# stelleg/caster-dta

Measured on AMD Instinct MI355X. Metric: graph-pairs/sec (Davis-shaped protein+drug), encoders fwd+bwd, higher is better.
Workload: dtype f32; 1 GPU; davis_b64; pairs_per_gpu=64, residues_per_gpu=19200, protein_edges_per_gpu=57484, atoms_per_gpu=2560, drug_edges_per_gpu=7986, encoder=CASTER-DTA(2,2), pass=fwdbwd, activation_storage=fp32, scope=encoders, torch_compile=False, tunable_gemms=False, two_lane_head=False, train_mode=True, csr_build_in_step=True, hip_graph=True, kernels=mfma

## Files before the change

caster-dta_amd/csrc/gvp_internal.h:

```cpp
#pragma once
#include <hip/hip_runtime.h>
#include <stdint.h>

#include "../../include/caster_gvp.h"
#include "gvp_math.h"
#include "gvp_rng.h"

constexpr int POLICY_F32 = 0, POLICY_BF16 = 1, POLICY_GVPDEF = 2, POLICY_LINEAR = 3;

struct QuadOffsets {
  int emb, conv0, node0, layer_stride, head, total;
  int embT, convT0, nodeT0, layerT_stride, headT;
};

#ifndef CGVP_BWD_MAX_GRID
#define CGVP_BWD_MAX_GRID 240
#endif
constexpr int kBwdMaxGrid = CGVP_BWD_MAX_GRID;

#include <atomic>
#include <type_traits>

template <auto Kernel, class... A>
int launch_reserving(dim3 grid, dim3 block, size_t lds, size_t reserve, hipStream_t st, const A&... args) {
// ... 14 lines not shown
  return 0;
}
template <auto Kernel, class... A>
int launch(dim3 grid, dim3 block, size_t lds, hipStream_t st, const A&... args) {
  return launch_reserving<Kernel>(grid, block, lds, lds, st, args...);
}

namespace gq { struct bf16s; struct f32_gvpdef; struct f32_linear; }
template <class T> struct Tag { using type = T; };
template <class ST> constexpr bool is_layer_kind = std::is_same_v<ST, gq::f32_gvpdef> || std::is_same_v<ST, gq::f32_linear>;
template <bool KINDS, class F>
int with_policy(int policy, F&& f) {
  if (policy == POLICY_F32) return f(Tag<float>{});
  if (policy == POLICY_BF16) return f(Tag<gq::bf16s>{});
  if constexpr (KINDS) {
    if (policy == POLICY_GVPDEF) return f(Tag<gq::f32_gvpdef>{});
    if (policy == POLICY_LINEAR) return f(Tag<gq::f32_linear>{});
  }
  return CGVP_ERR_UNSUPPORTED_DIMS;
}
template <class F>
int with_flag(bool b, F&& f) { return b ? f(std::true_type{}) : f(std::false_type{}); }

namespace quad {
int offsets(int nt_node, int nt_edge, int num_convs, QuadOffsets* o);
int prepare(const gvp::EncLayout& L, int num_convs, int packed_bf16, const float* params, float* image, hipStream_t st);
int node_embed(int nt_node, const float* img, const float* x_s, const float* x_v, const int64_t* ntypes,
               int64_t N, float* h, unsigned long long* rng_state, unsigned long long* rng_out, int policy, hipStream_t st);
int pass_begin(const gvp::EncLayout& L, int num_convs, int policy, const float* params, float* image, const float* x_s,
               const float* x_v, const int64_t* ntypes, int64_t N, float* h, unsigned long long* rng_state,
               unsigned long long* rng_out, const int64_t* edge_index, int64_t E, int32_t* counters, hipStream_t st);
int conv(int nt_edge, const float* img, const float* h, const float* e_s, const float* e_v,
         const int64_t* etypes, const int32_t* rowptr, const int32_t* eperm, const int32_t* esrc,
         const int32_t* edst, int64_t N, int64_t E, int mean, float* dh, int fuse, const float* img_node,
         const float* img_head, float* h_out, float* out, const float* mask0, const float* mask1, gvp::RngArgs rng,
         const float* e_in, float* e_out, int policy, hipStream_t st);
int node_update(const float* img_node, const float* img_head, const float* h, const float* dh, int64_t N,
                int with_head, float* h_out, float* out, const float* mask0, const float* mask1, gvp::RngArgs rng,
                int policy, hipStream_t st);

int node_update_bwd(const float* img_node, const float* imgT_node, const float* h, const float* dh,
                    const float* mask0, const float* mask1, gvp::RngArgs rng, const float* g_up0, const float* g_up1,
                    const float* g_up2, int64_t N, float* g_dh, float* g_h, float* zero_rows, float* slab, int* grid,
                    int policy, hipStream_t st);
int head_bwd(const float* img_head, const float* imgT_head, const float* h_out, const float* g_out, int64_t N,
             float* g_h_out, float* slab, int* grid, int policy, hipStream_t st);
int node_head_bwd(const float* img_head, const float* imgT_head, const float* h_out, const float* g_out, float* g_h_out,
                  float* head_slab, const float* img_node, const float* imgT_node, const float* h, const float* dh,
                  const float* mask0, const float* mask1, gvp::RngArgs rng, int64_t N, float* g_dh, float* g_h,
                  float* zero_rows, float* slab, int* grid, int policy, hipStream_t st);
int conv_bwd(int nt_edge, const float* img, const float* imgT, const float* h, const float* e_emb,
             const int32_t* rowptr, const int32_t* esrc, const int32_t* edst, int64_t N, int64_t E, int mean,
             const float* g_dh, float* g_src, float* g_dst, float* g_e, float* slab, int* grid, int policy, hipStream_t st,
             float* g_edge = nullptr, float* slot = nullptr);
// ... 44 lines not shown
```

caster-dta_amd/csrc/gvp_kernels.hip:

```cpp
#include <hip/hip_runtime.h>
#include <stdlib.h>
#include <stdint.h>

#include "gvp_internal.h"

using namespace gvp;

namespace {

constexpr int WAVE = 64;

inline int check_dims(const cgvp_dims* d) {
  if (!d) return CGVP_ERR_BAD_ARG;
  if (d->node_in_s != NODE_IN_S || d->node_in_v != NODE_IN_V || d->edge_in_s != EDGE_IN_S ||
      d->edge_in_v != EDGE_IN_V || d->hidden_s != NS || d->hidden_v != NV ||
      d->edge_hidden_s != ES || d->edge_hidden_v != EV || d->out_s != OUT)
    return CGVP_ERR_UNSUPPORTED_DIMS;
  if (d->storage != CGVP_F32 && d->storage != CGVP_BF16) return CGVP_ERR_UNSUPPORTED_DIMS;
  if (d->layer_kind < CGVP_LAYER_GATED || d->layer_kind > CGVP_LAYER_LINEAR) return CGVP_ERR_UNSUPPORTED_DIMS;
  if (d->layer_kind != CGVP_LAYER_GATED && d->storage != CGVP_F32) return CGVP_ERR_UNSUPPORTED_DIMS;
  return 0;
}
inline int check_dims_gated(const cgvp_dims* d) {
  if (int rc = check_dims(d)) return rc;
// ... 21 lines not shown

struct BwdLookup : QuadOffsets { quad::BwdBlocks blk; };
inline int bwd_lookup(const cgvp_layout& l, BwdLookup* o) {
  if (int rc = quad::offsets(l.nt_node, l.nt_edge, num_convs_of(l), o)) return rc;
  return quad::bwd_block_sizes(l.nt_node, l.nt_edge, &o->blk);
}
inline int emit_segments(const cgvp_segment* sg, int n, cgvp_segment* segs, int32_t* nsegs, float* grad_params,
                         hipStream_t st, int overwrite = 0, bool store_only = false) {
  if (segs && nsegs) { for (int k = 0; k < n; ++k) segs[k] = sg[k]; *nsegs = n; }
  else quad::reduce_segments(sg, n, grad_params, st, overwrite, store_only);
  return launch_status();
}

__global__ void zero_words_kernel(uint32_t* __restrict__ p, size_t n) {
  for (size_t i = (size_t)blockIdx.x * blockDim.x + threadIdx.x; i < n; i += (size_t)gridDim.x * blockDim.x) p[i] = 0u;
}
inline void zero_words(void* p, size_t words, hipStream_t s) {
  if (words == 0 || !p) return;
  size_t blocks = (words + 1023) / 1024;
  if (blocks > 2048) blocks = 2048;
  hipLaunchKernelGGL(zero_words_kernel, dim3((unsigned)blocks), dim3(256), 0, s, reinterpret_cast<uint32_t*>(p), words);
}

__global__ void csr_count_kernel(const int64_t* __restrict__ ei, int64_t N, int64_t E,
                                 int32_t* __restrict__ cnt, unsigned long long* rng_state, unsigned long long* rng_out) {
  int64_t e = (int64_t)blockIdx.x * blockDim.x + threadIdx.x;
  if (rng_state && e == 0) {
    const unsigned long long off = rng_state[1] + 1;
    rng_state[1] = off;
    rng_out[0] = rng_state[0];
    rng_out[1] = off;
  }
  if (e >= E) return;
  int64_t s = ei[e], d = ei[E + e];
  if (s < 0 || s >= N || d < 0 || d >= N) return;
  atomicAdd(&cnt[d], 1);
}

constexpr int SCAN_LDS = 36 * 1024;
__global__ __launch_bounds__(1024) void csr_scan_kernel(const int32_t* __restrict__ cnt, int64_t N,
                                                        int32_t* __restrict__ rowptr) {
  extern __shared__ int32_t sbuf[];
  const int t = threadIdx.x;
  const int tile_cap = (int)(N < SCAN_LDS ? (N + 3) / 4 * 4 : SCAN_LDS);
  int32_t* part = sbuf + tile_cap;
  int32_t carry = 0;
  for (int64_t base = 0; base < N || base == 0; base += SCAN_LDS) {
    const int64_t rem = N - base;
    const int n = (int)(rem < SCAN_LDS ? (rem > 0 ? rem : 0) : SCAN_LDS);
    constexpr int VPT = SCAN_LDS / 4096;
    int4 v[VPT];
    const int n4 = n >> 2;
    const int4* src4 = reinterpret_cast<const int4*>(cnt + base);
#pragma unroll
    for (int k = 0; k < VPT; ++k) {
      const int q = t + 1024 * k;
      v[k] = q < n4 ? src4[q] : make_int4(0, 0, 0, 0);
    }
#pragma unroll
// ... 26 lines not shown
    }
    __syncthreads();
    const int32_t wave_base = (t >> 6) > 0 ? part[16 + (t >> 6) - 1] : 0;
    const int32_t total = part[31];
    int32_t run = carry + wave_base + inc - sum;
    for (int i = lo; i < hi; ++i) { const int32_t c = sbuf[i]; sbuf[i] = run; run += c; }
    __syncthreads();
    if ((((uintptr_t)(rowptr + base)) & 15) == 0) {
      for (int q = t; q < n4; q += 1024) {
        const int4 x = reinterpret_cast<const int4*>(sbuf)[q];
        reinterpret_cast<int4*>(rowptr + base)[q] = x;
      }
      if (t < (n & 3)) rowptr[base + (n4 << 2) + t] = sbuf[(n4 << 2) + t];
    } else {
      for (int i = t; i < n; i += 1024) rowptr[base + i] = sbuf[i];
    }
    carry += total;
    __syncthreads();
    if (N == 0) break;
  }
  if (t == 0) rowptr[N] = carry;
}

constexpr int SCAN_MULTI_MAX = 65536, SCAN_MULTI_T = 256, SCAN_MULTI_CHUNK = 4 * SCAN_MULTI_T;
__global__ __launch_bounds__(SCAN_MULTI_T) void csr_scan_multi_kernel(const int32_t* __restrict__ cnt, int32_t N,
                                                                      int32_t counters, int32_t* __restrict__ rowptr) {
  __shared__ int32_t part[2 * (SCAN_MULTI_T / WAVE)];
  const int t = threadIdx.x, wv = t >> 6;
  const int4* c4 = reinterpret_cast<const int4*>(cnt);
  int32_t pre = 0;
  for (int q = t; q < (int)blockIdx.x * SCAN_MULTI_T; q += SCAN_MULTI_T) {
    const int4 v = c4[q];
    pre += (v.x + v.y) + (v.z + v.w);
  }
  const int i0 = (int)blockIdx.x * SCAN_MULTI_CHUNK + 4 * t;
  const int4 v = i0 < counters ? c4[i0 >> 2] : make_int4(0, 0, 0, 0);
  const int32_t sum = (v.x + v.y) + (v.z + v.w);
  int32_t inc = sum;
#pragma unroll
  for (int off = 1; off < WAVE; off <<= 1) {
    const int32_t u = __shfl_up(inc, off);
    if ((t & (WAVE - 1)) >= off) inc += u;
    pre += __shfl_xor(pre, off);
  }
  if ((t & (WAVE - 1)) == WAVE - 1) { part[wv] = inc; part[SCAN_MULTI_T / WAVE + wv] = pre; }
  __syncthreads();
  int32_t run = inc - sum;
// ... 21 lines not shown
  tmp[pos] = (int32_t)e;
  edst[pos] = (int32_t)d;
}

__global__ void csr_rank_kernel(const int64_t* __restrict__ ei, int64_t N, int64_t E, int64_t counters,
                                const int32_t* __restrict__ rowptr, const int32_t* __restrict__ tmp,
                                int32_t* __restrict__ edst, int32_t* __restrict__ eperm,
                                int32_t* __restrict__ esrc, int32_t* __restrict__ cnt) {
  const int64_t t = (int64_t)blockIdx.x * blockDim.x + threadIdx.x;
  if (t < counters) cnt[t] = 0;
  if (t >= rowptr[N] || t >= E) {
    if (t < E) { eperm[t] = -1; esrc[t] = 0; edst[t] = 0; }
    return;
  }
  const int32_t n = edst[t];
  if (n < 0 || n >= N) return;
  int32_t lo = rowptr[n], hi = rowptr[n + 1];
  const int32_t key = tmp[t];
  if (lo < 0 || hi > E || lo > hi || key < 0 || key >= E) return;
  int32_t rank = 0;
  for (int32_t j = lo; j < hi; ++j) rank += tmp[j] < key ? 1 : 0;
  eperm[lo + rank] = key;
  esrc[lo + rank] = (int32_t)ei[key];
}

__global__ void src_count_kernel(const int32_t* __restrict__ esrc, const int32_t* __restrict__ rowptr, int64_t N,
                                 int32_t* __restrict__ cnt) {
  const int64_t p = (int64_t)blockIdx.x * blockDim.x + threadIdx.x;
  if (p >= rowptr[N]) return;
  const int32_t s = esrc[p];
  if (s >= 0 && s < N) atomicAdd(&cnt[s], 1);
}
__global__ void src_fill_kernel(const int32_t* __restrict__ esrc, const int32_t* __restrict__ rowptr, int64_t N,
                                const int32_t* __restrict__ sptr, int32_t* __restrict__ cnt, int32_t* __restrict__ tmp) {
  const int64_t p = (int64_t)blockIdx.x * blockDim.x + threadIdx.x;
  const int32_t ev = rowptr[N];
  if (p >= ev) return;
  const int32_t s = esrc[p];
  if (s < 0 || s >= N) return;
  const int32_t pos = sptr[s] + atomicSub(&cnt[s], 1) - 1;
  if (pos >= 0 && pos < ev) tmp[pos] = (int32_t)p;
}
__global__ void src_rank_kernel(const int32_t* __restrict__ esrc, const int32_t* __restrict__ rowptr, int64_t N,
                                const int32_t* __restrict__ sptr, const int32_t* __restrict__ tmp, int32_t* __restrict__ spos) {
  const int64_t k = (int64_t)blockIdx.x * blockDim.x + threadIdx.x;
  const int32_t ev = rowptr[N];
// ... 370 lines not shown
    if (a.width == 20) {
      if (blk < 4) {
        float fs[4], fv;
        gvp::dropout_row20(a.rng.seed[0], a.rng.seed[1], a.rng.stream + m, n, blk, a.rng.p, fs, fv);
        row[4 * blk] = fs[0]; row[4 * blk + 1] = fs[1]; row[4 * blk + 2] = fs[2]; row[4 * blk + 3] = fs[3];
        row[16 + blk] = fv;
      }
    } else {
      float f[4];
      gvp::dropout4(a.rng.seed[0], a.rng.seed[1], a.rng.stream + m, n, blk, a.rng.p, f);
      row[4 * blk] = f[0]; row[4 * blk + 1] = f[1]; row[4 * blk + 2] = f[2]; row[4 * blk + 3] = f[3];
    }
  }
}

extern "C" {

int cgvp_abi_version(void) { return CGVP_ABI_VERSION; }
const char* cgvp_build_info(void) { return "libcaster_gvp gfx950 (HIP, wave64), built " __DATE__ " " __TIME__; }

int cgvp_csr_from_coo(const int64_t* edge_index, int64_t N, int64_t E, int32_t* rowptr,
                      int32_t* eperm, int32_t* esrc, int32_t* edst, int32_t* work, int32_t work_is_zero,
                      int32_t* ids_scratch, void* stream) {
  return quad::csr_build(edge_index, N, E, rowptr, eperm, esrc, edst, work, work_is_zero, ids_scratch, nullptr, nullptr,
                         (hipStream_t)stream);
}
}

namespace quad {
void zero_words(void* p, size_t words, hipStream_t s) { ::zero_words(p, words, s); }

int csr_build(const int64_t* edge_index, int64_t N, int64_t E, int32_t* rowptr, int32_t* eperm, int32_t* esrc,
              int32_t* edst, int32_t* work, int work_is_zero, int32_t* ids_scratch, unsigned long long* rng_state,
              unsigned long long* rng_out, hipStream_t stream) {
  if (N < 0 || E < 0 || !rowptr || !work || (E > 0 && (!edge_index || !eperm || !esrc || !edst || !ids_scratch)))
    return CGVP_ERR_BAD_ARG;
  if (N >= (int64_t)1 << 31 || E >= (int64_t)1 << 31) return CGVP_ERR_BAD_ARG;
  if ((uintptr_t)work & 15) return CGVP_ERR_BAD_ARG;
  hipStream_t s = stream;
  const int64_t counters = (N + 1 + 63) / 64 * 64;
  if (work_is_zero == 0) {
    zero_words(work, (size_t)counters, s);
  }
  int32_t* tmp = ids_scratch;
  const int B = 256;
  if (E > 0 && work_is_zero != 2)
    hipLaunchKernelGGL(csr_count_kernel, dim3((unsigned)((E + B - 1) / B)), dim3(B), 0, s, edge_index, N, E, work, rng_state, rng_out);
  else if (rng_state)
    hipLaunchKernelGGL(rng_next_kernel, dim3(1), dim3(1), 0, s, rng_state, rng_out);
  if (N < SCAN_MULTI_MAX) {
    hipLaunchKernelGGL(csr_scan_multi_kernel, dim3((unsigned)((N + 1 + SCAN_MULTI_CHUNK - 1) / SCAN_MULTI_CHUNK)),
                       dim3(SCAN_MULTI_T), 0, s, work, (int32_t)N, (int32_t)counters, rowptr);
  } else {
    const int64_t tile = N < SCAN_LDS ? (N + 3) / 4 * 4 : SCAN_LDS;
    hipLaunchKernelGGL(csr_scan_kernel, dim3(1), dim3(1024), (size_t)(tile + 1024 + 32) * sizeof(int32_t), s, work, N, rowptr);
  }
  if (E > 0) hipLaunchKernelGGL(csr_fill_kernel, dim3((unsigned)((E + B - 1) / B)), dim3(B), 0, s, edge_index, N, E, rowptr, work, tmp, edst);
  const int64_t span = E > counters ? E : counters;
  hipLaunchKernelGGL(csr_rank_kernel, dim3((unsigned)((span + B - 1) / B)), dim3(B), 0, s, edge_index, N, E, counters, rowptr, tmp,
                     edst, eperm, esrc, work);
  return launch_status();
}

bool deterministic_env() {
  static const bool v = [] { const char* e = getenv("CGVP_DETERMINISTIC"); return e && e[0] == '1'; }();
  return v;
}

int64_t src_index_work_ints(int64_t N, int64_t E) { return (N + 1 + 63) / 64 * 64 + (E > 0 ? E : 1); }

int src_index(const int32_t* rowptr, const int32_t* esrc, int64_t N, int64_t E, int32_t* sptr, int32_t* spos,
              int32_t* work, hipStream_t s) {
  if (N < 0 || E < 0 || !rowptr || !sptr || !work || (E > 0 && (!esrc || !spos))) return CGVP_ERR_BAD_ARG;
  if (N >= (int64_t)1 << 31 || E >= (int64_t)1 << 31 || ((uintptr_t)work & 15)) return CGVP_ERR_BAD_ARG;
  const int64_t counters = (N + 1 + 63) / 64 * 64;
  int32_t* cnt = work;
  int32_t* tmp = work + counters;
  zero_words(cnt, (size_t)counters, s);
  const int B = 256;
  const unsigned eb = (unsigned)((E + B - 1) / B);
// ... 41 lines not shown
  return 0;
}

int64_t cgvp_lba_image_floats(const cgvp_dims* dims, const cgvp_layout* layout) {
  if (int rc = check_dims(dims)) return rc;
  if (!layout) return CGVP_ERR_BAD_ARG;
  QuadOffsets o;
  if (int rc = quad::offsets(layout->nt_node, layout->nt_edge, num_convs_of(*layout), &o)) return rc;
  return o.total;
}

int cgvp_lba_prepare(const cgvp_dims* dims, const cgvp_layout* layout, const float* params, float* image,
                     void* stream) {
  if (int rc = check_dims(dims)) return rc;
  if (!layout || !params || !image) return CGVP_ERR_BAD_ARG;
  if (int rc = quad::prepare(cvt(*layout), num_convs_of(*layout), policy_of(dims) == POLICY_BF16 ? 1 : 0, params, image, (hipStream_t)stream)) return rc;
  return launch_status();
}

int cgvp_lba_pass_begin(const cgvp_dims* dims, const cgvp_layout* layout, const float* params, float* image,
                        const float* x_s, const float* x_v, const int64_t* ntypes, int64_t N, float* h,
                        uint64_t* rng_state, uint64_t* rng_out, const int64_t* edge_index, int64_t E,
                        int32_t* csr_counters, void* stream) {
  if (int rc = check_dims_gated(dims)) return rc;
  if (N < 0 || E < 0 || !layout || !params || !image || (layout->nt_node > 0 && N > 0 && !ntypes)) return CGVP_ERR_BAD_ARG;
  if ((rng_state != nullptr) != (rng_out != nullptr)) return CGVP_ERR_BAD_ARG;
  if (((uintptr_t)rng_state & 7) || ((uintptr_t)rng_out & 7) || ((uintptr_t)h & 15) || ((uintptr_t)image & 15)) return CGVP_ERR_BAD_ARG;
  if ((edge_index != nullptr) != (csr_counters != nullptr)) return CGVP_ERR_BAD_ARG;
  if (N > 0 && (!x_s || !x_v || !h)) return CGVP_ERR_BAD_ARG;
  if (N >= (int64_t)1 << 31 || E >= (int64_t)1 << 31) return CGVP_ERR_BAD_ARG;
  if (N == 0 && rng_state)
    if (int rc = cgvp_rng_next(rng_state, rng_out, stream)) return rc;
  if (int rc = quad::pass_begin(cvt(*layout), num_convs_of(*layout), policy_of(dims), params, image, x_s, x_v, ntypes, N, h,
                                reinterpret_cast<unsigned long long*>(rng_state), reinterpret_cast<unsigned long long*>(rng_out),
                                edge_index, E, csr_counters, (hipStream_t)stream)) return rc;
  return launch_status();
}


int cgvp_node_embed_fwd(const cgvp_dims* dims, const cgvp_layout* layout, const float* params,
                        const float* image, const float* x_s, const float* x_v, const int64_t* ntypes,
                        int64_t N, float* h, uint64_t* rng_state, uint64_t* rng_out, void* stream) {
  if (int rc = check_dims_gated(dims)) return rc;
  if (N < 0 || !layout || !params || (layout->nt_node > 0 && N > 0 && !ntypes)) return CGVP_ERR_BAD_ARG;
  if ((rng_state != nullptr) != (rng_out != nullptr) || (rng_state && !image)) return CGVP_ERR_BAD_ARG;
  if (((uintptr_t)rng_state & 7) || ((uintptr_t)rng_out & 7)) return CGVP_ERR_BAD_ARG;
  if (N == 0) return rng_state ? cgvp_rng_next(rng_state, rng_out, stream) : 0;
  if (!x_s || !x_v || !h) return CGVP_ERR_BAD_ARG;
  if (image) {
    if ((uintptr_t)h & 15) return CGVP_ERR_BAD_ARG;
    QuadOffsets o;
    if (int rc = quad::offsets(layout->nt_node, layout->nt_edge, num_convs_of(*layout), &o)) return rc;
    if (int rc = quad::node_embed(layout->nt_node, image + o.emb, x_s, x_v, ntypes, N, h,
                                  reinterpret_cast<unsigned long long*>(rng_state),
                                  reinterpret_cast<unsigned long long*>(rng_out), policy_of(dims), (hipStream_t)stream)) return rc;
    return launch_status();
  }
  if (policy_of(dims)) return CGVP_ERR_UNSUPPORTED_DIMS;
  NodeEmbedArgs a{params, cvt(*layout), x_s, x_v, ntypes, N, h};
  const dim3 grid((unsigned)((N + WAVE - 1) / WAVE));
  hipStream_t st = (hipStream_t)stream;
// ... 380 lines not shown
```

caster-dta_amd/csrc/gvp_quad_kernels.hip:

```cpp
#include <hip/hip_runtime.h>
#include <stdlib.h>
#include <stdint.h>

#include "gvp_internal.h"
#include "gvp_quad.h"

using namespace gq;

namespace {

#ifdef CGVP_STAMPS
__device__ unsigned long long* g_stamp_buf = nullptr;
#define STAMP(slot)                                                                          \
  do {                                                                                       \
    __builtin_amdgcn_sched_barrier(0);                                                       \
    unsigned long long t_;                                                                   \
    asm volatile("s_waitcnt vmcnt(0) lgkmcnt(0)\n\ts_memtime %0\n\ts_waitcnt lgkmcnt(0)" : "=s"(t_)::"memory"); \
    __builtin_amdgcn_sched_barrier(0);                                                       \
    if (g_stamp_buf && (threadIdx.x & 63) == 0)                                              \
      g_stamp_buf[((size_t)blockIdx.x * WPB + (threadIdx.x >> 6)) * 16 + (slot)] = t_;        \
  } while (0)
#define STAMP_REAL(slot)                                                                     \
  do {                                                                                       \
    unsigned long long t_;                                                                   \
// ... 124 lines not shown
  int type[1] = {0};
#pragma unroll
  for (int s = 0; s < Q::SSTEPS; ++s) {
    const int c = 4 * s + g;
    bs[0][s] = (active && c < NODE_IN_S) ? Io<ST>::ld(a.x_s, n * NODE_IN_S + c) : 0.f;
  }
#pragma unroll
  for (int p = 0; p < 3; ++p) bv[0][p][0] = (active && g < NODE_IN_V) ? Io<ST>::ld(a.x_v, n * 3 * NODE_IN_V + 3 * g + p) : 0.f;
  if (NTN > 0 && active) {
    type[0] = (int)a.ntypes[n];
    type[0] = type[0] < 0 ? 0 : (type[0] >= NTN ? NTN - 1 : type[0]);
  }
  f4 s[1][1];
  float v[1][3][1];
  typename Q::Cache c[1];
  Q::template forward<1, Io<ST>::BF>(lds + IM::EMB_GVP, lane, type, bs, bv, s, v, c);
  ln_quad<NS, NV>(lds + IM::EMB_LN, lane, s[0], v[0]);
  if (active) {
    Io<ST>::st4(a.h, n * ROW + 4 * g, s[0][0]);
#pragma unroll
    for (int p = 0; p < 3; ++p) Io<ST>::st(a.h, n * ROW + NS + 3 * g + p, v[0][p][0]);
  }
}
__device__ __forceinline__ void rng_handoff(const EmbedQArgs& a) {
  if (a.rng_state && blockIdx.x == 0 && threadIdx.x == 0) {
    const unsigned long long off = a.rng_state[1] + 1;
    a.rng_state[1] = off;
    a.rng_out[0] = a.rng_state[0];
    a.rng_out[1] = off;
  }
}

template <int NTN, typename ST>
__global__ __launch_bounds__(TPB) void embed_quad_kernel(EmbedQArgs a) {
  typedef Image<NTN, 0> IM;
  __shared__ __attribute__((aligned(16))) float lds[IM::EMB_SIZE];
  stage_slice<IM::EMB_SIZE>(lds, a.img, threadIdx.x);
  rng_handoff(a);
  __syncthreads();
  embed_tile<NTN, ST>(a, lds, blockIdx.x);
}

struct PassBeginArgs {
  EmbedQArgs e;
  const float* params; EncLayout L; int num_convs; int packed; float* image;
  const int64_t* ei; int64_t E; int64_t Ncount; int32_t* counters;
  int embed_blocks, prep_blocks;
};
template <int NTN, int NTE, typename ST>
__global__ __launch_bounds__(TPB) void pass_begin_kernel(PassBeginArgs a) {
  typedef Image<NTN, NTE> IM;
  __shared__ __attribute__((aligned(16))) float lds[IM::EMB_SIZE];
  const int b = blockIdx.x;
  if (b >= a.embed_blocks + a.prep_blocks) {
    const int64_t e = (int64_t)(b - a.embed_blocks - a.prep_blocks) * TPB + threadIdx.x;
    if (e < a.E) {
      const int64_t s = a.ei[e], d = a.ei[a.E + e];
      if (s >= 0 && s < a.Ncount && d >= 0 && d < a.Ncount) atomicAdd(&a.counters[d], 1);
    }
    return;
  }
  if (b >= a.embed_blocks) {
    const int total = IM::total(a.num_convs);
    for (int idx = (b - a.embed_blocks) * TPB + threadIdx.x; idx < total; idx += a.prep_blocks * TPB)
      a.image[idx] = image_element<NTN, NTE>(a.params, a.L, a.num_convs, a.packed, idx);
    return;
  }
  for (int k = threadIdx.x; k < IM::EMB_SIZE; k += TPB) lds[k] = image_element<NTN, NTE>(a.params, a.L, a.num_convs, a.packed, k);
  rng_handoff(a.e);
  __syncthreads();
  embed_tile<NTN, ST>(a.e, lds, b);
}

struct NodeQArgs {
  const float* img_node; const float* img_head;
  const float* h; const float* dh; int64_t N; float* h_out; float* out;
  const float* mask0; const float* mask1;
  gvp::RngArgs rng;
};
constexpr int MROW = NS + NV;

__device__ __forceinline__ void node_dropout(const float* mask, const gvp::RngArgs& rng, int which, int64_t n, int g,
                                             f4& ms, float& mv) {
  if (mask) {
    ms = *reinterpret_cast<const f4*>(mask + n * MROW + 4 * g);
    mv = mask[n * MROW + NS + g];
  } else if (rng.seed) {
    const unsigned long long seed = rng.seed[0], off = rng.seed[1];
    float fs[4];
    gvp::dropout_row20(seed, off, rng.stream + which, n, g, rng.p, fs, mv);
    ms = f4{fs[0], fs[1], fs[2], fs[3]};
  }
// ... 414 lines not shown
int node_embed(int nt_node, const float* img, const float* x_s, const float* x_v, const int64_t* ntypes,
               int64_t N, float* h, unsigned long long* rng_state, unsigned long long* rng_out, int policy, hipStream_t st) {
  EmbedQArgs a{img, x_s, x_v, ntypes, N, h, rng_state, rng_out};
  const dim3 grid((unsigned)((N + WPB * TILE - 1) / (WPB * TILE)));
  return with_policy<false>(policy, [&](auto tag) {
    using ST = typename decltype(tag)::type;
    switch (nt_node) {
      case 0: return launch<embed_quad_kernel<0, ST>>(grid, dim3(TPB), 0, st, a);
      case 20: return launch<embed_quad_kernel<20, ST>>(grid, dim3(TPB), 0, st, a);
      case 21: return launch<embed_quad_kernel<21, ST>>(grid, dim3(TPB), 0, st, a);
      default: return CGVP_ERR_UNSUPPORTED_DIMS;
    }
  });
}

template <int NTN, int NTE>
int pass_begin_impl(const PassBeginArgs& a, int blocks, int policy, hipStream_t st) {
  return with_policy<false>(policy, [&](auto tag) {
    return launch<pass_begin_kernel<NTN, NTE, typename decltype(tag)::type>>(dim3(blocks), dim3(TPB), 0, st, a);
  });
}
int pass_begin(const EncLayout& L, int num_convs, int policy, const float* params, float* image, const float* x_s,
               const float* x_v, const int64_t* ntypes, int64_t N, float* h, unsigned long long* rng_state,
               unsigned long long* rng_out, const int64_t* edge_index, int64_t E, int32_t* counters, hipStream_t st) {
  QuadOffsets o;
  if (int rc = offsets(L.nt_node, L.nt_edge, num_convs, &o)) return rc;
  PassBeginArgs a{};
  a.e = EmbedQArgs{nullptr, x_s, x_v, ntypes, N, h, rng_state, rng_out};
  a.params = params; a.L = L; a.num_convs = num_convs; a.packed = policy == POLICY_BF16 ? 1 : 0; a.image = image;
  a.ei = edge_index; a.E = (edge_index && counters) ? E : 0; a.Ncount = N; a.counters = counters;
  a.embed_blocks = (int)((N + WPB * TILE - 1) / (WPB * TILE));
  a.prep_blocks = (o.total + TPB - 1) / TPB;
  const int blocks = a.embed_blocks + a.prep_blocks + (int)((a.E + TPB - 1) / TPB);
  return with_nt(L.nt_node, L.nt_edge, [&](auto ntn, auto nte) {
    return pass_begin_impl<decltype(ntn)::value, decltype(nte)::value>(a, blocks, policy, st);
  });
}

inline int conv_fwd_waves(int64_t groups) {
  static const int forced = [] { const char* e = getenv("CGVP_CONV_FWD_WAVES"); return (e && e[0] == '4') ? 4 : ((e && e[0] == '8') ? 8 : 0); }();
  if (forced) return forced;
  return groups <= 8 * (int64_t)kBwdMaxGrid ? 8 : 4;
}
template <int NTE, int FUSE, int EMODE, typename ST, int CW>
int conv_launch_w(const ConvQArgs& a, int64_t groups, hipStream_t st) {
  const size_t lds = (size_t)(Image<0, NTE>::CV_SIZE + (FUSE == 0 ? 0 : Image<0, 0>::ND_SIZE + (FUSE == 2 ? Image<0, 0>::HD_SIZE : 0)) +
                              CW * WAVE * ROW) * sizeof(float);
  return launch<conv_quad_kernel<NTE, FUSE, EMODE, ST, CW>>(dim3((unsigned)((groups + CW - 1) / CW)), dim3(WAVE * CW), lds, st, a);
}
template <int NTE, int FUSE, int EMODE, typename ST>
int conv_launch_e(const ConvQArgs& a, int64_t groups, hipStream_t st) {
  if (conv_fwd_waves(groups) == 4) return conv_launch_w<NTE, FUSE, EMODE, ST, 4>(a, groups, st);
  return conv_launch_w<NTE, FUSE, EMODE, ST, 8>(a, groups, st);
}
template <int NTE, int FUSE, typename ST>
int conv_launch_s(const ConvQArgs& a, int64_t grid, hipStream_t st) {
// ... 64 lines not shown
```

caster-dta_amd/csrc/pass_api.hip:

```cpp
#include <hip/hip_runtime.h>
#include <stdint.h>
#include <stdlib.h>

#include <atomic>
#include <mutex>
#include <vector>

#include "gvp_internal.h"

namespace {

struct TimedLaunch { hipEvent_t a, b; int kind; };
std::atomic<bool> g_timing{false};
std::mutex g_timed_mutex;
std::vector<TimedLaunch> g_timed;
struct Timed {
  hipStream_t st; bool on; TimedLaunch t;
  Timed(int kind, void* stream) : st((hipStream_t)stream), on(g_timing.load(std::memory_order_relaxed)) {
    if (!on) return;
    t.kind = kind;
    if (hipEventCreate(&t.a) != hipSuccess || hipEventCreate(&t.b) != hipSuccess) { on = false; return; }
    (void)hipEventRecord(t.a, st);
  }
  ~Timed() {
// ... 192 lines not shown
  if (int rc = cgvp_lba_fwd_workspace(dims, layout, N, E, save_state, &ws)) return rc;
  const int nc = num_convs_of(*layout);
  if (nc < 1) return CGVP_ERR_UNSUPPORTED_DIMS;
  if (!(dropout_p >= 0.f && dropout_p < 1.f)) return CGVP_ERR_BAD_ARG;
  const bool drop = dropout_p > 0.f && save_state;
  const bool draw = drop && !masks;
  if (draw && !rng_state) return CGVP_ERR_BAD_ARG;
  const bool tables = has_tables(batch);
  if (tables && (E > 0 && (!batch->eperm || !batch->esrc || !batch->edst))) return CGVP_ERR_BAD_ARG;
  if (!tables && E > 0 && (!batch->edge_index || !csr_counters)) return CGVP_ERR_BAD_ARG;
  if (N > 0 && !out) return CGVP_ERR_BAD_ARG;
  const int es = esize(dims);
  float* image = at<float>(workspace, ws.image);
  uint64_t* seed = at<uint64_t>(workspace, ws.seed);
  char* state = at<char>(workspace, ws.state);
  const int64_t srow = ws.node_stride * ROW * es;
  auto row = [&](int64_t r) { return reinterpret_cast<float*>(state + r * srow); };
  float* e_emb = at<float>(workspace, ws.e_emb);
  int32_t* rowptr = tables ? const_cast<int32_t*>(batch->rowptr) : at<int32_t>(workspace, ws.rowptr);
  int32_t* eperm = tables ? const_cast<int32_t*>(batch->eperm) : at<int32_t>(workspace, ws.eperm);
  int32_t* esrc = tables ? const_cast<int32_t*>(batch->esrc) : at<int32_t>(workspace, ws.esrc);
  int32_t* edst = tables ? const_cast<int32_t*>(batch->edst) : at<int32_t>(workspace, ws.edst);
  const bool count_here = !tables && E > 0;
  if (int rc = cgvp_lba_pass_begin(dims, layout, params, image, batch->x_s, batch->x_v, batch->ntypes, N, row(0),
                                   draw ? rng_state : nullptr, draw ? seed : nullptr,
                                   count_here ? batch->edge_index : nullptr, E, count_here ? csr_counters : nullptr, stream))
    return rc;
  if (!tables) {
    if (!csr_counters) return CGVP_ERR_BAD_ARG;
    if (int rc = cgvp_csr_from_coo(batch->edge_index, N, E, rowptr, eperm, esrc, edst, csr_counters, count_here ? 2 : 1,
                                   at<int32_t>(workspace, ws.ids_scratch), stream))
      return rc;
  }
  if (N == 0) return 0;
  int32_t fuse_i = 0;
  (void)cgvp_lba_forward_plan(N, E, nc, tables ? 1 : 0, flags, &fuse_i);
  const bool fuse = fuse_i != 0;
  const int64_t mstride = N * MROW;
  for (int l = 0; l < nc; ++l) {
    const bool last = l == nc - 1;
    cgvp_rng rng{draw ? seed : nullptr, dropout_p, 2 * l};
    const cgvp_rng* rp = draw ? &rng : nullptr;
    const float* m0 = (drop && masks) ? masks + (int64_t)(2 * l) * mstride : nullptr;
    const float* m1 = (drop && masks) ? masks + (int64_t)(2 * l + 1) * mstride : nullptr;
    float *h, *dh, *h_out;
    if (save_state) { h = row(l); dh = row(nc + l); h_out = last ? row(2 * nc) : row(l + 1); }
    else { h = row(l & 1); dh = fuse ? nullptr : row(2); h_out = last ? nullptr : row((l + 1) & 1); }
    const float* e_in = l > 0 ? e_emb : nullptr;
    float* e_out = l == 0 ? e_emb : nullptr;
    if (fuse) {
      Timed timed(0, stream);
      if (int rc = cgvp_conv_layer_fwd(dims, layout, image, l, h, batch->e_s, batch->e_v, batch->etypes, rowptr, eperm, esrc,
                                       edst, N, E, aggr_mean, m0, m1, rp, last ? 1 : 0, e_in, e_out, dh, h_out, out, stream))
        return rc;
// ... 368 lines not shown
```

Baseline: 281,000 graph-pairs/sec.

## Fuse CSR prefix scan into count kernel and fill with segment ranking

```diff
diff --git a/caster-dta_amd/csrc/gvp_internal.h b/caster-dta_amd/csrc/gvp_internal.h
--- a/caster-dta_amd/csrc/gvp_internal.h
+++ b/caster-dta_amd/csrc/gvp_internal.h
@@ -60,6 +60,69 @@
 template <class F>
 int with_flag(bool b, F&& f) { return b ? f(std::true_type{}) : f(std::false_type{}); }
 
+constexpr int SCAN_MULTI_MAX = 65536;
+constexpr int CSR_FUSED_RANK_MAX_E = 65535;
+constexpr int CSR_WORK_SCANNED = 3;
+constexpr int CSR_TAIL_T = 256, CSR_TAIL_LDS = 3 * (CSR_TAIL_T / 64);
+#ifdef __HIPCC__
+__device__ __forceinline__ void csr_count_tail(int32_t* cnt, int32_t N, int count_blocks, int32_t* rowptr, int32_t* part) {
+  constexpr int NW = CSR_TAIL_T / 64;
+  const int t = threadIdx.x, ln = t & 63, wv = t >> 6;
+  asm volatile("s_waitcnt vmcnt(0)" ::: "memory");
+  __syncthreads();
+  if (t == 0) {
+    __builtin_amdgcn_fence(__ATOMIC_RELEASE, "agent");
+    asm volatile("s_waitcnt vmcnt(0)" ::: "memory");
+    const int ticket = __hip_atomic_fetch_add(&cnt[N], 1, __ATOMIC_RELAXED, __HIP_MEMORY_SCOPE_AGENT);
+    const int last = ticket == count_blocks - 1;
+    if (last) {
+      __hip_atomic_store(&cnt[N], 0, __ATOMIC_RELAXED, __HIP_MEMORY_SCOPE_AGENT);
+      __builtin_amdgcn_fence(__ATOMIC_ACQUIRE, "agent");
+      asm volatile("s_waitcnt vmcnt(0)" ::: "memory");
+    }
+    part[2 * NW] = last;
+  }
+  __syncthreads();
+  if (!part[2 * NW]) return;
+  const int4* c4 = reinterpret_cast<const int4*>(cnt);
+  const int passes = (N + 1 + 4 * CSR_TAIL_T - 1) / (4 * CSR_TAIL_T);
+  int32_t carry = 0;
+  int4 nxt = 4 * t <= N ? c4[t] : make_int4(0, 0, 0, 0);
+  for (int p = 0; p < passes; ++p) {
+    const int i0 = (p * CSR_TAIL_T + t) * 4;
+    int4 v = nxt;
+    const int i1 = i0 + 4 * CSR_TAIL_T;
+    nxt = (p + 1 < passes && i1 <= N) ? c4[i1 >> 2] : make_int4(0, 0, 0, 0);
+    int32_t x[4] = {v.x, v.y, v.z, v.w};
+#pragma unroll
+    for (int k = 0; k < 4; ++k) if (i0 + k >= N) x[k] = 0;
+    const int32_t sum = (x[0] + x[1]) + (x[2] + x[3]);
+    int32_t inc = sum;
+#pragma unroll
+    for (int off = 1; off < 64; off <<= 1) {
+      const int32_t u = __shfl_up(inc, off);
+      if (ln >= off) inc += u;
+    }
+    int32_t* pp = part + (p & 1) * NW;
+    if (ln == 63) pp[wv] = inc;
+    __syncthreads();
+    int32_t run = carry + inc - sum, total = 0;
+#pragma unroll
+    for (int w = 0; w < NW; ++w) {
+      const int32_t pw = pp[w];
+      total += pw;
+      if (w < wv) run += pw;
+    }
+    carry += total;
+#pragma unroll
+    for (int k = 0; k < 4; ++k) {
+      if (i0 + k <= N) rowptr[i0 + k] = run;
+      run += x[k];
+    }
+  }
+}
+#endif
+
 namespace quad {
 int offsets(int nt_node, int nt_edge, int num_convs, QuadOffsets* o);
 int prepare(const gvp::EncLayout& L, int num_convs, int packed_bf16, const float* params, float* image, hipStream_t st);
@@ -67,7 +130,11 @@
                int64_t N, float* h, unsigned long long* rng_state, unsigned long long* rng_out, int policy, hipStream_t st);
 int pass_begin(const gvp::EncLayout& L, int num_convs, int policy, const float* params, float* image, const float* x_s,
                const float* x_v, const int64_t* ntypes, int64_t N, float* h, unsigned long long* rng_state,
-               unsigned long long* rng_out, const int64_t* edge_index, int64_t E, int32_t* counters, hipStream_t st);
+               unsigned long long* rng_out, const int64_t* edge_index, int64_t E, int32_t* counters, int32_t* rowptr,
+               int* scanned, hipStream_t st);
+int pass_begin_entry(const cgvp_dims* dims, const cgvp_layout* layout, const float* params, float* image, const float* x_s,
+                     const float* x_v, const int64_t* ntypes, int64_t N, float* h, uint64_t* rng_state, uint64_t* rng_out,
+                     const int64_t* edge_index, int64_t E, int32_t* csr_counters, int32_t* rowptr, int* scanned, void* stream);
 int conv(int nt_edge, const float* img, const float* h, const float* e_s, const float* e_v,
          const int64_t* etypes, const int32_t* rowptr, const int32_t* eperm, const int32_t* esrc,
          const int32_t* edst, int64_t N, int64_t E, int mean, float* dh, int fuse, const float* img_node,
diff --git a/caster-dta_amd/csrc/gvp_kernels.hip b/caster-dta_amd/csrc/gvp_kernels.hip
--- a/caster-dta_amd/csrc/gvp_kernels.hip
+++ b/caster-dta_amd/csrc/gvp_kernels.hip
@@ -67,8 +67,10 @@
   hipLaunchKernelGGL(zero_words_kernel, dim3((unsigned)blocks), dim3(256), 0, s, reinterpret_cast<uint32_t*>(p), words);
 }
 
-__global__ void csr_count_kernel(const int64_t* __restrict__ ei, int64_t N, int64_t E,
-                                 int32_t* __restrict__ cnt, unsigned long long* rng_state, unsigned long long* rng_out) {
+__global__ __launch_bounds__(CSR_TAIL_T) void csr_count_kernel(const int64_t* __restrict__ ei, int64_t N, int64_t E,
+                                                               int32_t* cnt, unsigned long long* rng_state,
+                                                               unsigned long long* rng_out, int32_t* rowptr) {
+  __shared__ int32_t part[CSR_TAIL_LDS];
   int64_t e = (int64_t)blockIdx.x * blockDim.x + threadIdx.x;
   if (rng_state && e == 0) {
     const unsigned long long off = rng_state[1] + 1;
@@ -76,10 +78,11 @@
     rng_out[0] = rng_state[0];
     rng_out[1] = off;
   }
-  if (e >= E) return;
-  int64_t s = ei[e], d = ei[E + e];
-  if (s < 0 || s >= N || d < 0 || d >= N) return;
-  atomicAdd(&cnt[d], 1);
+  if (e < E) {
+    int64_t s = ei[e], d = ei[E + e];
+    if (s >= 0 && s < N && d >= 0 && d < N) atomicAdd(&cnt[d], 1);
+  }
+  if (rowptr) csr_count_tail(cnt, (int32_t)N, (int)gridDim.x, rowptr, part);
 }
 
 constexpr int SCAN_LDS = 36 * 1024;
@@ -152,7 +155,7 @@
   if (t == 0) rowptr[N] = carry;
 }
 
-constexpr int SCAN_MULTI_MAX = 65536, SCAN_MULTI_T = 256, SCAN_MULTI_CHUNK = 4 * SCAN_MULTI_T;
+constexpr int SCAN_MULTI_T = 256, SCAN_MULTI_CHUNK = 4 * SCAN_MULTI_T;
 __global__ __launch_bounds__(SCAN_MULTI_T) void csr_scan_multi_kernel(const int32_t* __restrict__ cnt, int32_t N,
                                                                       int32_t counters, int32_t* __restrict__ rowptr) {
   __shared__ int32_t part[2 * (SCAN_MULTI_T / WAVE)];
@@ -220,6 +223,73 @@
   for (int32_t j = lo; j < hi; ++j) rank += tmp[j] < key ? 1 : 0;
   eperm[lo + rank] = key;
   esrc[lo + rank] = (int32_t)ei[key];
+}
+
+#ifndef CGVP_RANK_LANE_MAX
+#define CGVP_RANK_LANE_MAX 16
+#endif
+constexpr int RANK_LANE_MAX = CGVP_RANK_LANE_MAX;
+__global__ __launch_bounds__(256) void csr_fill_rank_kernel(const int64_t* __restrict__ ei, int64_t N, int32_t E,
+                                                            const int32_t* __restrict__ rowptr, int32_t* cnt, int32_t* tmp,
+                                                            int32_t* edst, int32_t* eperm, int32_t* esrc) {
+  const int32_t e = (int32_t)(blockIdx.x * 256 + threadIdx.x);
+  const int lane = threadIdx.x & (WAVE - 1);
+  int32_t d = 0, lo = 0, hi = 0;
+  bool stored = false;
+  if (e < E) {
+    const int64_t s = ei[e], dd = ei[(int64_t)E + e];
+    if (s >= 0 && s < N && dd >= 0 && dd < N) {
+      d = (int32_t)dd;
+      lo = rowptr[d]; hi = rowptr[d + 1];
+      const uint32_t old = (uint32_t)__hip_atomic_fetch_add(&cnt[d], -1, __ATOMIC_RELAXED, __HIP_MEMORY_SCOPE_AGENT);
+      const int32_t pos = lo + (int32_t)(old & 0xffffu) - 1;
+      if (lo >= 0 && hi <= E && lo <= hi && pos >= 0 && pos < E) {
+        tmp[pos] = e;
+        edst[pos] = d;
+        stored = true;
+      }
+    }
+  }
+  __builtin_amdgcn_fence(__ATOMIC_RELEASE, "agent");
+  asm volatile("s_waitcnt vmcnt(0)" ::: "memory");
+  bool mine = false;
+  if (stored) {
+    const uint32_t old = (uint32_t)__hip_atomic_fetch_add(&cnt[d], 1 << 16, __ATOMIC_RELAXED, __HIP_MEMORY_SCOPE_AGENT);
+    mine = (int32_t)(old >> 16) + 1 == hi - lo;
+    if (mine) __hip_atomic_store(&cnt[d], 0, __ATOMIC_RELAXED, __HIP_MEMORY_SCOPE_AGENT);
+  }
+  __builtin_amdgcn_fence(__ATOMIC_ACQUIRE, "agent");
+  if (e < E && e >= rowptr[N]) { eperm[e] = -1; esrc[e] = 0; edst[e] = 0; }
+  if (mine && hi - lo <= RANK_LANE_MAX) {
+    for (int32_t p = lo; p < hi; ++p) {
+      const int32_t key = tmp[p];
+      if (key < 0 || key >= E) continue;
+      int32_t rank = 0;
+      for (int32_t j = lo; j < hi; ++j) rank += tmp[j] < key ? 1 : 0;
+      eperm[lo + rank] = key;
+      esrc[lo + rank] = (int32_t)ei[key];
+    }
+  }
+  unsigned long long big = __ballot(mine && hi - lo > RANK_LANE_MAX);
+  while (big) {
+    const int leader = __ffsll(big) - 1;
+    big &= big - 1;
+    const int32_t slo = __shfl(lo, leader), shi = __shfl(hi, leader);
+    for (int32_t p0 = slo; p0 < shi; p0 += WAVE) {
+      const int32_t p = p0 + lane;
+      const int32_t key = p < shi ? tmp[p] : INT32_MAX;
+      int32_t rank = 0;
+      for (int32_t j0 = slo; j0 < shi; j0 += WAVE) {
+        const int32_t v = j0 + lane < shi ? tmp[j0 + lane] : INT32_MAX;
+#pragma unroll
+        for (int k = 0; k < WAVE; ++k) rank += __builtin_amdgcn_readlane(v, k) < key ? 1 : 0;
+      }
+      if (p < shi && key >= 0 && key < E) {
+        eperm[slo + rank] = key;
+        esrc[slo + rank] = (int32_t)ei[key];
+      }
+    }
+  }
 }
 
 __global__ void src_count_kernel(const int32_t* __restrict__ esrc, const int32_t* __restrict__ rowptr, int64_t N,
@@ -636,8 +706,8 @@
 int cgvp_csr_from_coo(const int64_t* edge_index, int64_t N, int64_t E, int32_t* rowptr,
                       int32_t* eperm, int32_t* esrc, int32_t* edst, int32_t* work, int32_t work_is_zero,
                       int32_t* ids_scratch, void* stream) {
-  return quad::csr_build(edge_index, N, E, rowptr, eperm, esrc, edst, work, work_is_zero, ids_scratch, nullptr, nullptr,
-                         (hipStream_t)stream);
+  return quad::csr_build(edge_index, N, E, rowptr, eperm, esrc, edst, work, (work_is_zero == 0 || work_is_zero == 2) ? work_is_zero : 1,
+                         ids_scratch, nullptr, nullptr, (hipStream_t)stream);
 }
 }
 
@@ -651,6 +721,7 @@
     return CGVP_ERR_BAD_ARG;
   if (N >= (int64_t)1 << 31 || E >= (int64_t)1 << 31) return CGVP_ERR_BAD_ARG;
   if ((uintptr_t)work & 15) return CGVP_ERR_BAD_ARG;
+  if (work_is_zero == CSR_WORK_SCANNED && !(E > 0 && N < SCAN_MULTI_MAX)) return CGVP_ERR_BAD_ARG;
   hipStream_t s = stream;
   const int64_t counters = (N + 1 + 63) / 64 * 64;
   if (work_is_zero == 0) {
@@ -658,18 +729,29 @@
   }
   int32_t* tmp = ids_scratch;
   const int B = 256;
-  if (E > 0 && work_is_zero != 2)
-    hipLaunchKernelGGL(csr_count_kernel, dim3((unsigned)((E + B - 1) / B)), dim3(B), 0, s, edge_index, N, E, work, rng_state, rng_out);
+  static_assert(B == CSR_TAIL_T, "csr_count_kernel's scan tail is written for this workgroup size");
+  const unsigned eblocks = (unsigned)((E + B - 1) / B);
+  const bool count_here = E > 0 && work_is_zero != 2 && work_is_zero != CSR_WORK_SCANNED;
+  const bool scan_in_count = count_here && N < SCAN_MULTI_MAX;
+  if (count_here)
+    hipLaunchKernelGGL(csr_count_kernel, dim3(eblocks), dim3(B), 0, s, edge_index, N, E, work, rng_state, rng_out,
+                       scan_in_count ? rowptr : nullptr);
   else if (rng_state)
     hipLaunchKernelGGL(rng_next_kernel, dim3(1), dim3(1), 0, s, rng_state, rng_out);
-  if (N < SCAN_MULTI_MAX) {
+  if (scan_in_count || work_is_zero == CSR_WORK_SCANNED) {
+  } else if (N < SCAN_MULTI_MAX) {
     hipLaunchKernelGGL(csr_scan_multi_kernel, dim3((unsigned)((N + 1 + SCAN_MULTI_CHUNK - 1) / SCAN_MULTI_CHUNK)),
                        dim3(SCAN_MULTI_T), 0, s, work, (int32_t)N, (int32_t)counters, rowptr);
   } else {
     const int64_t tile = N < SCAN_LDS ? (N + 3) / 4 * 4 : SCAN_LDS;
     hipLaunchKernelGGL(csr_scan_kernel, dim3(1), dim3(1024), (size_t)(tile + 1024 + 32) * sizeof(int32_t), s, work, N, rowptr);
   }
-  if (E > 0) hipLaunchKernelGGL(csr_fill_kernel, dim3((unsigned)((E + B - 1) / B)), dim3(B), 0, s, edge_index, N, E, rowptr, work, tmp, edst);
+  if (E > 0 && E <= CSR_FUSED_RANK_MAX_E) {
+    hipLaunchKernelGGL(csr_fill_rank_kernel, dim3(eblocks), dim3(B), 0, s, edge_index, N, (int32_t)E, rowptr, work, tmp, edst,
+                       eperm, esrc);
+    return launch_status();
+  }
+  if (E > 0) hipLaunchKernelGGL(csr_fill_kernel, dim3(eblocks), dim3(B), 0, s, edge_index, N, E, rowptr, work, tmp, edst);
   const int64_t span = E > counters ? E : counters;
   hipLaunchKernelGGL(csr_rank_kernel, dim3((unsigned)((span + B - 1) / B)), dim3(B), 0, s, edge_index, N, E, counters, rowptr, tmp,
                      edst, eperm, esrc, work);
@@ -757,21 +839,34 @@
                         const float* x_s, const float* x_v, const int64_t* ntypes, int64_t N, float* h,
                         uint64_t* rng_state, uint64_t* rng_out, const int64_t* edge_index, int64_t E,
                         int32_t* csr_counters, void* stream) {
+  return quad::pass_begin_entry(dims, layout, params, image, x_s, x_v, ntypes, N, h, rng_state, rng_out, edge_index, E,
+                                csr_counters, nullptr, nullptr, stream);
+}
+
+}
+
+int quad::pass_begin_entry(const cgvp_dims* dims, const cgvp_layout* layout, const float* params, float* image,
+                           const float* x_s, const float* x_v, const int64_t* ntypes, int64_t N, float* h,
+                           uint64_t* rng_state, uint64_t* rng_out, const int64_t* edge_index, int64_t E,
+                           int32_t* csr_counters, int32_t* rowptr, int* scanned, void* stream) {
+  if (scanned) *scanned = 0;
   if (int rc = check_dims_gated(dims)) return rc;
   if (N < 0 || E < 0 || !layout || !params || !image || (layout->nt_node > 0 && N > 0 && !ntypes)) return CGVP_ERR_BAD_ARG;
   if ((rng_state != nullptr) != (rng_out != nullptr)) return CGVP_ERR_BAD_ARG;
   if (((uintptr_t)rng_state & 7) || ((uintptr_t)rng_out & 7) || ((uintptr_t)h & 15) || ((uintptr_t)image & 15)) return CGVP_ERR_BAD_ARG;
   if ((edge_index != nullptr) != (csr_counters != nullptr)) return CGVP_ERR_BAD_ARG;
+  if (rowptr && ((uintptr_t)csr_counters & 15)) return CGVP_ERR_BAD_ARG;
   if (N > 0 && (!x_s || !x_v || !h)) return CGVP_ERR_BAD_ARG;
   if (N >= (int64_t)1 << 31 || E >= (int64_t)1 << 31) return CGVP_ERR_BAD_ARG;
   if (N == 0 && rng_state)
     if (int rc = cgvp_rng_next(rng_state, rng_out, stream)) return rc;
   if (int rc = quad::pass_begin(cvt(*layout), num_convs_of(*layout), policy_of(dims), params, image, x_s, x_v, ntypes, N, h,
                                 reinterpret_cast<unsigned long long*>(rng_state), reinterpret_cast<unsigned long long*>(rng_out),
-                                edge_index, E, csr_counters, (hipStream_t)stream)) return rc;
-  return launch_status();
-}
-
+                                edge_index, E, csr_counters, rowptr, scanned, (hipStream_t)stream)) return rc;
+  return launch_status();
+}
+
+extern "C" {
 
 int cgvp_node_embed_fwd(const cgvp_dims* dims, const cgvp_layout* layout, const float* params,
                         const float* image, const float* x_s, const float* x_v, const int64_t* ntypes,
diff --git a/caster-dta_amd/csrc/gvp_quad_kernels.hip b/caster-dta_amd/csrc/gvp_quad_kernels.hip
--- a/caster-dta_amd/csrc/gvp_quad_kernels.hip
+++ b/caster-dta_amd/csrc/gvp_quad_kernels.hip
@@ -170,8 +170,8 @@
     for (int p = 0; p < 3; ++p) Io<ST>::st(a.h, n * ROW + NS + 3 * g + p, v[0][p][0]);
   }
 }
-__device__ __forceinline__ void rng_handoff(const EmbedQArgs& a) {
-  if (a.rng_state && blockIdx.x == 0 && threadIdx.x == 0) {
+__device__ __forceinline__ void rng_handoff(const EmbedQArgs& a, int block) {
+  if (a.rng_state && block == 0 && threadIdx.x == 0) {
     const unsigned long long off = a.rng_state[1] + 1;
     a.rng_state[1] = off;
     a.rng_out[0] = a.rng_state[0];
@@ -184,7 +184,7 @@
   typedef Image<NTN, 0> IM;
   __shared__ __attribute__((aligned(16))) float lds[IM::EMB_SIZE];
   stage_slice<IM::EMB_SIZE>(lds, a.img, threadIdx.x);
-  rng_handoff(a);
+  rng_handoff(a, blockIdx.x);
   __syncthreads();
   embed_tile<NTN, ST>(a, lds, blockIdx.x);
 }
@@ -192,30 +192,33 @@
 struct PassBeginArgs {
   EmbedQArgs e;
   const float* params; EncLayout L; int num_convs; int packed; float* image;
-  const int64_t* ei; int64_t E; int64_t Ncount; int32_t* counters;
-  int embed_blocks, prep_blocks;
+  const int64_t* ei; int64_t E; int64_t Ncount; int32_t* counters; int32_t* rowptr;
+  int count_blocks, embed_blocks;
 };
+static_assert(TPB == CSR_TAIL_T, "csr_count_tail is written for the workgroup size of pass_begin_kernel");
 template <int NTN, int NTE, typename ST>
 __global__ __launch_bounds__(TPB) void pass_begin_kernel(PassBeginArgs a) {
   typedef Image<NTN, NTE> IM;
   __shared__ __attribute__((aligned(16))) float lds[IM::EMB_SIZE];
-  const int b = blockIdx.x;
-  if (b >= a.embed_blocks + a.prep_blocks) {
-    const int64_t e = (int64_t)(b - a.embed_blocks - a.prep_blocks) * TPB + threadIdx.x;
+  if ((int)blockIdx.x < a.count_blocks) {
+    const int64_t e = (int64_t)blockIdx.x * TPB + threadIdx.x;
     if (e < a.E) {
       const int64_t s = a.ei[e], d = a.ei[a.E + e];
       if (s >= 0 && s < a.Ncount && d >= 0 && d < a.Ncount) atomicAdd(&a.counters[d], 1);
     }
+    if (a.rowptr) csr_count_tail(a.counters, (int32_t)a.Ncount, a.count_blocks, a.rowptr, reinterpret_cast<int32_t*>(lds));
     return;
   }
+  const int b = (int)blockIdx.x - a.count_blocks;
   if (b >= a.embed_blocks) {
     const int total = IM::total(a.num_convs);
-    for (int idx = (b - a.embed_blocks) * TPB + threadIdx.x; idx < total; idx += a.prep_blocks * TPB)
+    const int prep_blocks = (int)gridDim.x - a.count_blocks - a.embed_blocks;
+    for (int idx = (b - a.embed_blocks) * TPB + threadIdx.x; idx < total; idx += prep_blocks * TPB)
       a.image[idx] = image_element<NTN, NTE>(a.params, a.L, a.num_convs, a.packed, idx);
     return;
   }
   for (int k = threadIdx.x; k < IM::EMB_SIZE; k += TPB) lds[k] = image_element<NTN, NTE>(a.params, a.L, a.num_convs, a.packed, k);
-  rng_handoff(a.e);
+  rng_handoff(a.e, b);
   __syncthreads();
   embed_tile<NTN, ST>(a.e, lds, b);
 }
@@ -676,16 +679,19 @@
 }
 int pass_begin(const EncLayout& L, int num_convs, int policy, const float* params, float* image, const float* x_s,
                const float* x_v, const int64_t* ntypes, int64_t N, float* h, unsigned long long* rng_state,
-               unsigned long long* rng_out, const int64_t* edge_index, int64_t E, int32_t* counters, hipStream_t st) {
+               unsigned long long* rng_out, const int64_t* edge_index, int64_t E, int32_t* counters, int32_t* rowptr,
+               int* scanned, hipStream_t st) {
   QuadOffsets o;
   if (int rc = offsets(L.nt_node, L.nt_edge, num_convs, &o)) return rc;
   PassBeginArgs a{};
   a.e = EmbedQArgs{nullptr, x_s, x_v, ntypes, N, h, rng_state, rng_out};
   a.params = params; a.L = L; a.num_convs = num_convs; a.packed = policy == POLICY_BF16 ? 1 : 0; a.image = image;
   a.ei = edge_index; a.E = (edge_index && counters) ? E : 0; a.Ncount = N; a.counters = counters;
+  a.count_blocks = (int)((a.E + TPB - 1) / TPB);
+  a.rowptr = (a.count_blocks > 0 && N < SCAN_MULTI_MAX) ? rowptr : nullptr;
+  if (scanned) *scanned = a.rowptr != nullptr;
   a.embed_blocks = (int)((N + WPB * TILE - 1) / (WPB * TILE));
-  a.prep_blocks = (o.total + TPB - 1) / TPB;
-  const int blocks = a.embed_blocks + a.prep_blocks + (int)((a.E + TPB - 1) / TPB);
+  const int blocks = a.count_blocks + a.embed_blocks + (o.total + TPB - 1) / TPB;
   return with_nt(L.nt_node, L.nt_edge, [&](auto ntn, auto nte) {
     return pass_begin_impl<decltype(ntn)::value, decltype(nte)::value>(a, blocks, policy, st);
   });
diff --git a/caster-dta_amd/csrc/pass_api.hip b/caster-dta_amd/csrc/pass_api.hip
--- a/caster-dta_amd/csrc/pass_api.hip
+++ b/caster-dta_amd/csrc/pass_api.hip
@@ -238,14 +238,17 @@
   int32_t* esrc = tables ? const_cast<int32_t*>(batch->esrc) : at<int32_t>(workspace, ws.esrc);
   int32_t* edst = tables ? const_cast<int32_t*>(batch->edst) : at<int32_t>(workspace, ws.edst);
   const bool count_here = !tables && E > 0;
-  if (int rc = cgvp_lba_pass_begin(dims, layout, params, image, batch->x_s, batch->x_v, batch->ntypes, N, row(0),
-                                   draw ? rng_state : nullptr, draw ? seed : nullptr,
-                                   count_here ? batch->edge_index : nullptr, E, count_here ? csr_counters : nullptr, stream))
+  int scanned = 0;
+  if (int rc = quad::pass_begin_entry(dims, layout, params, image, batch->x_s, batch->x_v, batch->ntypes, N, row(0),
+                                      draw ? rng_state : nullptr, draw ? seed : nullptr,
+                                      count_here ? batch->edge_index : nullptr, E, count_here ? csr_counters : nullptr,
+                                      count_here ? rowptr : nullptr, &scanned, stream))
     return rc;
   if (!tables) {
     if (!csr_counters) return CGVP_ERR_BAD_ARG;
-    if (int rc = cgvp_csr_from_coo(batch->edge_index, N, E, rowptr, eperm, esrc, edst, csr_counters, count_here ? 2 : 1,
-                                   at<int32_t>(workspace, ws.ids_scratch), stream))
+    if (int rc = quad::csr_build(batch->edge_index, N, E, rowptr, eperm, esrc, edst, csr_counters,
+                                 scanned ? CSR_WORK_SCANNED : (count_here ? 2 : 1), at<int32_t>(workspace, ws.ids_scratch),
+                                 nullptr, nullptr, (hipStream_t)stream))
       return rc;
   }
   if (N == 0) return 0;
```

After: 232,900 graph-pairs/sec. -17.1%, worse.
